# lawfuyang/HobbyRenderer

Hardware: AMD Instinct MI355X
Metric: Mrays/s at 1920×1080, 8 spp, 4 bounces; 1/2/4/8 GPU scaling (higher is better)
Workload: dtype f32; 1 GPU; config 2: Cornell-box-class procedural scene (38 triangles, 9 instances, closed room, emissive quad + default sun), 1920x1080, 8 spp (accumulation indices 0..7), 4 bounces; frames_in_flight=2, serial_kernels=False, mode=default

## Files before the change

hobbyrenderer_amd/csrc/pt_capi.cpp:

```cpp
#include <mutex>

#include "pt_capi_internal.h"

using namespace hrt;
using namespace hrt::capi;

static std::mutex g_errMutex;
static std::string g_createError;

int capi::fail(HrptContext* ctx, int code, const std::string& msg)
{
    if (ctx) ctx->err = msg;
    else { std::lock_guard<std::mutex> l(g_errMutex); g_createError = msg; }
    return code;
}

int capi::realloc_image(HrptContext* c, DeviceBuffer<float4>& image, size_t bytes)
{
    HIP_TRY(c, image.alloc(bytes));
    HIP_TRY(c, hipMemsetAsync(image, 0, bytes, c->stream));
    return HRPT_OK;
}

int hrpt_create(const HrptDeviceDesc* desc, HrptContext** out)
// ... 170 lines not shown
    c->accelStructure = structure;
    return HRPT_OK;
} catch (...) { return caught(c, "hrpt_set_acceleration_structure"); }

int hrpt_set_bvh_builder(HrptContext* c, int builder)
try {
    if (!c) return HRPT_ERR_INVALID_ARGUMENT;
    if (builder != HRPT_BVH_BUILDER_HOST_SAH && builder != HRPT_BVH_BUILDER_GPU_LBVH && builder != HRPT_BVH_BUILDER_GPU_PLOC && builder != HRPT_BVH_BUILDER_AUTO) return fail(c, HRPT_ERR_INVALID_ARGUMENT, "hrpt_set_bvh_builder: unknown builder");
    c->bvhBuilder = builder;
    return HRPT_OK;
} catch (...) { return caught(c, "hrpt_set_bvh_builder"); }

int hrpt_get_build_info(HrptContext* c, HrptBuildInfo* out)
try {
    if (!c) return HRPT_ERR_INVALID_ARGUMENT;
    if (!out) return fail(c, HRPT_ERR_INVALID_ARGUMENT, "hrpt_get_build_info: null out");
    if (!c->haveScene) return fail(c, HRPT_ERR_INVALID_ARGUMENT, "hrpt_get_build_info: no scene uploaded");
    *out = c->buildInfo;
    return HRPT_OK;
} catch (...) { return caught(c, "hrpt_get_build_info"); }

int hrpt_get_stats(HrptContext* c, HrptStats* out)
try {
    if (!c) return HRPT_ERR_INVALID_ARGUMENT;
    if (!out) return fail(c, HRPT_ERR_INVALID_ARGUMENT, "hrpt_get_stats: null out");
    HIP_TRY(c, hipSetDevice(c->device));
    HIP_TRY(c, hipStreamSynchronize(c->stream));
    DeviceCounters h[kCounterShards];
    HIP_TRY(c, hipMemcpy(h, c->perContext.dCounters, sizeof h, hipMemcpyDeviceToHost));
    memset(out, 0, sizeof *out);
    DeviceCounters total{};
    for (int i = 0; i < kCounterShards; ++i) {
        total.closestRays += h[i].closestRays; total.shadowRays += h[i].shadowRays; total.paths += h[i].paths; total.neeEntries += h[i].neeEntries;
        total.neeSamples += h[i].neeSamples; total.radianceShade += h[i].radianceShade; total.radianceShadow += h[i].radianceShadow; total.skipped16 += h[i].skipped16;
        total.fusedPaths += h[i].fusedPaths; total.fusedEntries += h[i].fusedEntries;
    }
    out->closestRays = total.closestRays; out->shadowRays = total.shadowRays; out->paths = total.paths;
    out->neeEntries = total.neeEntries; out->neeSamples = total.neeSamples;
    out->megakernelFallbacks = c->megakernelFallbacks; out->queuePoolBytes = c->wf.poolBytes;
    if (total.neeEntries || c->wf.raygenBytes || c->wf.resolveBytes) {
        wavefront_queue_bytes(c->wf, total, out->traceQueueBytes, out->shadeQueueBytes, out->shadowQueueBytes);
        out->raygenQueueBytes = c->wf.raygenBytes; out->resolveQueueBytes = c->wf.resolveBytes;
    }
    if (c->timed) { float ms = 0.0f; if (hipEventElapsedTime(&ms, c->evStart, c->evStop) == hipSuccess) out->lastRenderMs = ms; }
    wavefront_collect_timing(c->wf);
    out->traceKernelMs = c->wf.kernelMs[kKernelExtend]; out->traceKernelLaunches = c->wf.kernelLaunches[kKernelExtend];
    out->shadeKernelMs = c->wf.kernelMs[kKernelShade]; out->shadeKernelLaunches = c->wf.kernelLaunches[kKernelShade];
    out->shadowKernelMs = c->wf.kernelMs[kKernelShadow]; out->shadowKernelLaunches = c->wf.kernelLaunches[kKernelShadow];
    out->raygenKernelMs = c->wf.kernelMs[kKernelRaygen]; out->raygenKernelLaunches = c->wf.kernelLaunches[kKernelRaygen];
    out->resolveKernelMs = c->wf.kernelMs[kKernelResolve]; out->resolveKernelLaunches = c->wf.kernelLaunches[kKernelResolve];
    out->bvhNodeCount = c->bvhNodes; out->bvhTriangleCount = c->bvhTris; out->bvhMaxDepth = c->traits.bvhMaxDepth;
    return HRPT_OK;
} catch (...) { return caught(c, "hrpt_get_stats"); }

int hrpt_reset_stats(HrptContext* c)
try {
    if (!c) return HRPT_ERR_INVALID_ARGUMENT;
    HIP_TRY(c, hipSetDevice(c->device));
    HIP_TRY(c, hipStreamSynchronize(c->stream));
    HIP_TRY(c, hipMemsetAsync(c->perContext.dCounters, 0, sizeof(DeviceCounters) * kCounterShards, c->stream));
    wavefront_reset_timing(c->wf);
    c->megakernelFallbacks = 0;
    return HRPT_OK;
} catch (...) { return caught(c, "hrpt_reset_stats"); }
```

hobbyrenderer_amd/csrc/pt_kernels.h:

```cpp
#pragma once

#include <hip/hip_runtime.h>
#include <stdint.h>

#include "../../include/hobbyrt_pt.h"

namespace hrt {

struct SceneView;
struct MotionArgs;
struct GpuNode4; struct GpuNodeQ;

constexpr int kCounterShards = 32;
struct DeviceCounters {
    unsigned long long closestRays;
    unsigned long long shadowRays;
    unsigned long long paths;
    unsigned long long neeEntries;
    unsigned long long neeSamples;
    unsigned long long radianceShade;
    unsigned long long radianceShadow;
    unsigned long long skipped16;
    unsigned long long fusedPaths;
    unsigned long long fusedEntries;
};

struct TileRect {
    uint32_t x0, y0, x1, y1;
    uint32_t stripeCount = 1, stripeIndex = 0;
    __host__ __device__ uint32_t columns() const { uint32_t all = (x1 - x0 + 7u) / 8u; return all > stripeIndex ? (all - stripeIndex + stripeCount - 1u) / stripeCount : 0u; }
    __host__ __device__ uint32_t column_x(uint32_t k) const { return x0 + (k * stripeCount + stripeIndex) * 8u; }
};

hipError_t launch_megakernel(const SceneView& scene, const HrptPathTracerConstants& constants, float4* accumulation,
                             float4* output, uint32_t imageWidth, TileRect rect, DeviceCounters* counters, hipStream_t stream);

hipError_t launch_gbuffer_megakernel(const SceneView& scene, const HrptPathTracerConstants& constants, float4* const* planes, uint32_t planeMask,
                                     uint32_t imageWidth, TileRect rect, hipStream_t stream);

hipError_t launch_motion_megakernel(const SceneView& scene, const HrptPathTracerConstants& constants, float4* const* planes, uint32_t planeMask,
                                    const MotionArgs& motion, uint32_t imageWidth, TileRect rect, hipStream_t stream);

hipError_t launch_post_chain(const float4* hdr, float4* display, uint32_t pixelCount, const HrptPostParams& params, uint32_t* histogram,
                             float* exposure, hipStream_t stream);

size_t bloom_pyramid_words(uint32_t width, uint32_t height);
bool bloom_params_valid(const HrptBloomParams& params);
hipError_t launch_bloom(float4* hdr, uint32_t width, uint32_t height, const HrptBloomParams& params, uint32_t* downPyramid, uint32_t* upPyramid,
                        uint32_t tailTexels, hipStream_t stream);
void bloom_pack_probe(const float* rgb, uint32_t count, uint32_t* packed, float* unpacked);
void bloom_host(const float* hdrIn, float* hdrOut, uint32_t width, uint32_t height, const HrptBloomParams& params, int nthreads);

bool temporal_params_valid(const HrptTemporalParams& params);
hipError_t launch_temporal(const HrptTemporalImages& images, uint32_t width, uint32_t height, const HrptPlanarViewConstants& view,
                           const HrptPlanarViewConstants& prevView, const HrptTemporalParams& params, hipStream_t stream);
// ... 44 lines not shown
```

hobbyrenderer_amd/csrc/pt_wavefront.hip:

```cpp
#define HRPT_PHASE_TU 1
#include "pt_wavefront.h"

#include <mutex>
#include <type_traits>
#include <unordered_map>
#include <vector>

#include "bvh_build.h"
#include "pt_gbuffer.h"
#include "pt_motion.h"
#include "pt_path.h"

#ifdef HRPT_PHASE_PROFILE
__device__ unsigned long long g_phaseCounters[128];
#endif
#ifdef HRPT_SKY_DEBUG
__device__ float g_skyDebug[2048 * 16];
#endif

namespace hrt {

namespace {

#include "pt_wf_common.h"
// ... 184 lines not shown
        float t = 0.0f;
        if (hipEventElapsedTime(&t, st.events[i], st.events[i + 1]) == hipSuccess) { st.kernelMs[st.kind[i / 2]] += t; st.kernelLaunches[st.kind[i / 2]]++; }
    }
    st.eventsUsed = 0;
}

#ifdef HRPT_SKY_DEBUG
extern "C" int hrpt_sky_debug_read(float* out) { return hipMemcpyFromSymbol(out, HIP_SYMBOL(g_skyDebug), sizeof(float) * 2048 * 16) == hipSuccess ? 0 : -3; }
#endif
#ifdef HRPT_PHASE_PROFILE
extern "C" int hrpt_phase_profile_read(unsigned long long* out128)
{
    if (hipMemcpyFromSymbol(out128, HIP_SYMBOL(g_phaseCounters), 128 * sizeof(unsigned long long)) != hipSuccess) return -3;
    static const unsigned long long zero[128] = { 0 };
    if (hipMemcpyToSymbol(HIP_SYMBOL(g_phaseCounters), zero, sizeof zero) != hipSuccess) return -3;
    return 0;
}
#endif

void wavefront_reset_timing(WavefrontState& st)
{
    st.eventsUsed = 0;
    for (int k = 0; k < kKernelClasses; ++k) { st.kernelMs[k] = 0.0f; st.kernelLaunches[k] = 0; }
    st.raygenBytes = 0; st.resolveBytes = 0;
}

void wavefront_queue_bytes(const WavefrontState& st, const DeviceCounters& c, uint64_t& trace, uint64_t& shade, uint64_t& shadow)
{
    const uint64_t path = st.plan.pathRecordBytes, survivors = c.closestRays > c.paths ? c.closestRays - c.paths : 0;
    trace = c.closestRays * (32 + 16);
    shade = c.closestRays * (path + 16) + survivors * path + c.neeEntries * 80 + c.neeSamples * 16 + c.radianceShade * 32;
    shadow = c.neeEntries * 48 + c.neeSamples * 16 + c.radianceShadow * (32 + 32);
    if (st.plan.shadowMode == kShadowSlim) {
        shade = c.closestRays * (path + 16) + survivors * path + c.neeEntries * 32 + c.radianceShade * 32;
        shadow = c.neeEntries * (32 + 16) + c.radianceShadow * (16 + 32);
    }
    if (st.plan.shadowMode == kShadowResolve) shadow += c.neeEntries * 32 + c.neeSamples * 16 + c.shadowRays * 72 + c.neeEntries * st.plan.maxLights * 8;
    if (st.plan.fusedPrimary) {
        trace -= c.paths * 16;
        shade = shade - c.paths * (path - 16) + c.paths * 16;
        shadow -= c.skipped16 * 16;
        trace -= c.fusedPaths * 32;
        shade = shade - c.fusedPaths * 32 + c.fusedEntries * 16;
    }
}

namespace {
bool timing_mark(WavefrontState& st, hipStream_t stream, KernelClass kind, bool begin)
{
    if (st.eventsUsed >= 4096) return true;
    if (st.eventsUsed + 1 > st.events.size()) {
        hipEvent_t e;
        if (hipEventCreate(&e) != hipSuccess) return false;
        st.events.push_back(e);
    }
    if (begin) { if (st.kind.size() < st.eventsUsed / 2 + 1) st.kind.resize(st.eventsUsed / 2 + 1); st.kind[st.eventsUsed / 2] = (uint8_t)kind; }
    (void)hipEventRecord(st.events[st.eventsUsed], stream);
    st.eventsUsed++;
    return true;
}
struct PoolCarver {
    char* base; size_t off = 0;
    template <class T> void operator()(T*& stream, size_t bytes, bool present = true)
    {
        stream = reinterpret_cast<T*>(reinterpret_cast<uintptr_t>(base) + (present ? off : 0));
        if (present) off += (bytes + 255) & ~(size_t)255;
    }
};
size_t counter_bytes(uint64_t capacity) { return (size_t)(capacity / 64) * 4; }
void carve_paths_and_hits(PoolCarver& carve, WfBuffers& b, int queues, uint64_t capacity, bool hasMedium, bool hasInstances)
{
    for (int p = 0; p < queues; ++p) {
        carve(b.rayO[p], capacity * 16); carve(b.rayD[p], capacity * 16); carve(b.thr[p], capacity * 16);
        carve(b.med0[p], capacity * 16, hasMedium); carve(b.med1[p], capacity * 16, hasMedium);
        carve(b.pathCnt[p], counter_bytes(capacity));
    }
    carve(b.hit, capacity * 16);
    carve(b.hitInst, capacity * 4, hasInstances); if (!hasInstances) b.hitInst = nullptr;
}
size_t carve_pool(char* base, WfArgs& a, uint64_t capacity, uint32_t maxLights, const SceneTraits& traits, bool hasInstances)
{
    const bool hasShadowRayQueue = traits.hasNonOpaque || maxLights > 1;
    PoolCarver carve{ base };
    WfBuffers& b = a.b;
    carve_paths_and_hits(carve, b, 2, capacity, traits.hasMedium, hasInstances);
    carve(a.primaryArgs, sizeof(PrimaryArgs));
    carve(b.sh0, capacity * 16); carve(b.sh1, capacity * 16); carve(b.sh2, capacity * 16); carve(b.sh3, capacity * 16); carve(b.sh4, capacity * 16);
    carve(b.shL, capacity * 16 * maxLights);
    carve(b.shadowCnt, counter_bytes(capacity)); carve(b.radiance, capacity * 16);
    carve(b.sqO, capacity * 16 * maxLights, hasShadowRayQueue); carve(b.sqD, capacity * 16 * maxLights, hasShadowRayQueue); carve(b.sqId, capacity * 4 * maxLights, hasShadowRayQueue);
    carve(b.sqCnt, counter_bytes(capacity), hasShadowRayQueue); carve(b.shVis, capacity * 4 * maxLights, hasShadowRayQueue); carve(b.sqCand, capacity * 8 * kShadowCandidates * maxLights, hasShadowRayQueue);
    return carve.off;
}
size_t carve_gbuffer_pool(char* base, WfArgs& a, uint64_t capacity, bool hasMedium, bool hasInstances)
{
    PoolCarver carve{ base };
    carve_paths_and_hits(carve, a.b, 1, capacity, hasMedium, hasInstances);
    carve(a.b.radiance, capacity * 16);
    carve(a.counters, sizeof(DeviceCounters) * kCounterShards);
    return carve.off;
}
void fill_scene_args(WfArgs& a, const WavefrontState& st, const SceneView& scene, const SceneTraits& traits, TileRect rect, uint32_t width)
{
    a.scene = scene;
    a.tilesX = rect.columns(); a.tilesY = (rect.y1 - rect.y0 + 7) / 8; a.rect = rect; a.imageWidth = width; a.pixelsPadded = a.tilesX * a.tilesY * 64;
    a.hasMedium = traits.hasMedium ? 1u : 0u; a.hasStochasticAlpha = traits.hasStochasticAlpha ? 1u : 0u; a.allOpaque = traits.hasNonOpaque ? 0u : 1u;
    a.refillMin = st.knobs.refillMin ? st.knobs.refillMin : kRefillMinDefault; a.streamSegments = st.knobs.drainSegments ? 0u : 1u;
}
hipError_t size_batch_and_pool(WavefrontState& st, const RenderPlan& plan, const SceneTraits& traits, bool hasInstances, uint64_t pixelsPadded, uint32_t accumCount,
                               hipStream_t stream, WfArgs& a, uint32_t& sppPerBatch, std::string& error)
{
    sppPerBatch = accumCount < kMaxSppPerBatch ? accumCount : kMaxSppPerBatch;
    uint64_t maxSamples = 64ull << 20;
    if (pixelsPadded * sppPerBatch * plan.bytesPerSample > st.poolBytes) {
        size_t freeB = 0, totalB = 0;
        if (hipMemGetInfo(&freeB, &totalB) == hipSuccess) {
            const uint64_t budget = (uint64_t)(freeB + st.poolBytes) / 2;
            if (budget / plan.bytesPerSample < maxSamples) maxSamples = budget / plan.bytesPerSample;
        }
    }
// ... 153 lines not shown
```

hobbyrenderer_amd/csrc/pt_wf_common.h:

```cpp

constexpr uint32_t kMaxSppPerBatch = 64;

struct WfBuffers {
    float4 *rayO[2], *rayD[2], *thr[2], *med0[2], *med1[2];
    uint32_t* pathCnt[2];
    float4* hit;
    uint32_t* hitInst;
    float4 *sh0, *sh1, *sh2, *sh3, *sh4, *shL;
    uint32_t* shadowCnt;
    float4 *sqO, *sqD; uint32_t* sqId; uint32_t* sqCnt; uint32_t* shVis;
    uint2* sqCand;
    float4* radiance;
};

struct WfArgs {
    SceneView scene;
    WfBuffers b;
    uint32_t segSize;
    uint32_t numSegments;
    uint32_t numSamples;
    uint32_t pixelsPadded;
    uint32_t tilesX, tilesY;
    TileRect rect;
    uint32_t imageWidth;
    uint32_t spp;
    uint32_t maxLights;
    uint32_t hasMedium;
    uint32_t hasStochasticAlpha;
    uint32_t allOpaque;
    uint32_t refillMin;
    uint32_t streamSegments;
    uint32_t slimShadow;
    uint32_t shadowParity;
    uint32_t nodeLoopMin;
    uint32_t sortShade;
    uint32_t shadeInstances, shadeMaterials;
    const struct PrimaryArgs* primaryArgs;
    uint32_t primary;
    int32_t* spill[2];
    DeviceCounters* counters;
};
// ... 146 lines not shown
```

hobbyrenderer_amd/csrc/pt_wf_shade.h:

```cpp
template <int MAXL>
struct NeeBuf { float ux[MAXL], uy[MAXL]; uint32_t light[MAXL]; };

static_assert(sizeof(GpuTriAttr) == kTriAttrBytes && sizeof(GpuInstShade) == kInstShadeBytes && sizeof(HrptMaterialConstants) == kMaterialBytes, "pt_wavefront_plan.h shade_table_bytes");
HRT_DEV LdsShadeTables copy_shade_tables(char* dst, const WfArgs& a)
{
    const SceneView& s = a.scene;
    const uint32_t nA = s.triCount * (uint32_t)(sizeof(GpuTriAttr) / 16), nI = a.shadeInstances * (uint32_t)(sizeof(GpuInstShade) / 16);
    const uint32_t nM = a.shadeMaterials * (uint32_t)(sizeof(HrptMaterialConstants) / 4);
    float4* const dA = reinterpret_cast<float4*>(dst); float4* const dI = dA + nA; uint32_t* const dM = reinterpret_cast<uint32_t*>(dI + nI);
    const float4* const sA = reinterpret_cast<const float4*>(s.attrs); const float4* const sI = reinterpret_cast<const float4*>(s.instShade);
    const uint32_t* const sM = reinterpret_cast<const uint32_t*>(s.materials);
    for (uint32_t i = threadIdx.x; i < nA; i += kBlock) dA[i] = sA[i];
    for (uint32_t i = threadIdx.x; i < nI; i += kBlock) dI[i] = sI[i];
    for (uint32_t i = threadIdx.x; i < nM; i += kBlock) dM[i] = sM[i];
    LdsShadeTables t;
    t.attrs = (uint32_t)(uintptr_t)(LdsShadeTables::LdsPtr)dst; t.instShade = t.attrs + nA * 16u; t.materials = t.instShade + nI * 16u;
    return t;
}


struct ShadeLane { bool valid, inA; uint32_t slot; float4 o, d, t, ha; };
struct ShadeWave { uint32_t outCount = 0, shCount = 0, ringHead = 0, pending = 0; unsigned int nEntriesOut = 0, nRadiance = 0; };
template <int MAXL, bool SIMPLE, bool PRIMARY, uint32_t RING, bool FUSED, class TABLES>
HRT_DEV void shade_iteration(const WfArgs& a, const HrptPathTracerConstants& cb, const TABLES& tables, float* const ring, uint32_t in, uint32_t out, int bounce, int lastBounce,
                             const ShadeLane& L, uint32_t baseA, uint32_t baseB, bool endsA, ShadeWave& w, uint32_t& outCountB, uint32_t& shCountB)
{
    static_assert(!FUSED || (PRIMARY && SIMPLE && MAXL == 1), "wf_bounce0: the bounce-0 SIMPLE single-light body");
    static_assert((RING & (RING - 1u)) == 0u && RING >= 1u && RING <= 64u, "ring positions are masked; one flush takes at most 64 entries");
    constexpr uint32_t kRing = RING;
    const SceneView& s = a.scene;
    const uint32_t lane = lane_id();
    const bool inA = L.inA;
    uint32_t& outCount = w.outCount; uint32_t& shCount = w.shCount;
    outCountB = 0; shCountB = 0;
            bool valid = L.valid, alive = false, wantDefer = false, wantRadiance = false;
            LobeDraw ld; ld.spec = false; ld.specProb = 0.0f; ld.root = 0.0f; ld.sp = 0.0f; ld.cp = 0.0f;
            uint32_t nNee = 0, smp = 0, slotIn = 0;
            PathState ps; f3 neeT = mk3(0.0f, 0.0f, 0.0f);
            constexpr bool STREAMED = MAXL == 0;
            NeeBuf<(STREAMED ? 1 : MAXL)> nee; SurfaceCarry carry;
            if (valid) {
                HRT_PHASE(PH_SHADE_ITER);
                const uint32_t slot = L.slot;
                slotIn = slot;
                const float4 o = L.o, d = L.d, t = L.t, ha = L.ha;
                uint32_t tri = __float_as_uint(ha.w);
                const bool noPath = PRIMARY && tri == kNoPathRecord;
                if (tri < kNoPathRecord) tri &= 0x1FFFFFFFu;
                ps.ray.o = mk3(o.x, o.y, o.z); ps.ray.d = mk3(d.x, d.y, d.z); ps.ray.tmin = o.w; ps.ray.tmax = 1e10f;
                ps.rng = __float_as_uint(d.w);
                ps.throughput = mk3(t.x, t.y, t.z); smp = __float_as_uint(t.w);
                ps.radiance = mk3(0.0f, 0.0f, 0.0f);
                if (!SIMPLE && a.hasMedium) {
                    float4 m0 = a.b.med0[in][slot], m1 = a.b.med1[in][slot];
                    ps.sigmaA = mk3(m0.x, m0.y, m0.z); ps.interiorIOR = m0.w; ps.sigmaS = mk3(m1.x, m1.y, m1.z); ps.inVolume = m1.w != 0.0f;
                } else { ps.sigmaA = mk3(0.0f, 0.0f, 0.0f); ps.sigmaS = mk3(0.0f, 0.0f, 0.0f); ps.interiorIOR = 1.0f; ps.inVolume = false; }
                bool addRadiance = false; f3 add = mk3(0.0f, 0.0f, 0.0f);
                if (noPath) {
                } else if (tri != 0xFFFFFFFFu) {
                    HRT_PHASE(PH_SHADE_HIT);
// ... 27 lines not shown
                        g[6] = cb.m_SunDirection[0]; g[7] = cb.m_SunDirection[1]; g[8] = cb.m_SunDirection[2]; g[9] = s.lights[0].m_Intensity;
                        g[10] = ps.radiance.x; g[11] = ps.radiance.y; g[12] = ps.radiance.z; g[13] = ps.throughput.x; g[14] = ps.throughput.y; g[15] = ps.throughput.z;
                    }
#endif
                }
                if constexpr (PRIMARY) {
                    a.b.radiance[smp] = addRadiance ? make_float4(0.0f + add.x, 0.0f + add.y, 0.0f + add.z, 0.0f) : make_float4(0.0f, 0.0f, 0.0f, 0.0f);
                } else if (addRadiance) {
                    float4 r = a.b.radiance[smp];
                    r.x = r.x + add.x; r.y = r.y + add.y; r.z = r.z + add.z;
                    a.b.radiance[smp] = r;
                }
                if (lastBounce) alive = false;
                wantRadiance = addRadiance && !PRIMARY;
            }
            w.nRadiance += (unsigned int)__popcll(__ballot(wantRadiance));
            const unsigned long long mA = __ballot(alive && inA), mB = __ballot(alive && !inA);
            if (alive) {
                HRT_PHASE(PH_SHADE_WRITE);
                uint32_t o = inA ? baseA + outCount + prefix_rank(mA) : baseB + prefix_rank(mB);
                a.b.rayO[out][o] = make_float4(ps.ray.o.x, ps.ray.o.y, ps.ray.o.z, ps.ray.tmin);
                a.b.rayD[out][o] = make_float4(ps.ray.d.x, ps.ray.d.y, ps.ray.d.z, __uint_as_float(ps.rng));
                a.b.thr[out][o] = make_float4(ps.throughput.x, ps.throughput.y, ps.throughput.z, __uint_as_float(smp));
                if (!SIMPLE && a.hasMedium) {
                    a.b.med0[out][o] = make_float4(ps.sigmaA.x, ps.sigmaA.y, ps.sigmaA.z, ps.interiorIOR);
                    a.b.med1[out][o] = make_float4(ps.sigmaS.x, ps.sigmaS.y, ps.sigmaS.z, ps.inVolume ? 1.0f : 0.0f);
                }
            }
            const unsigned long long msA = __ballot(nNee > 0 && inA), msB = __ballot(nNee > 0 && !inA);
            if (SIMPLE && MAXL == 1 && a.slimShadow && nNee > 0) {
                uint32_t e = inA ? baseA + shCount + prefix_rank(msA) : baseB + prefix_rank(msB);
                a.b.sh0[e] = make_float4(carry.worldPos.x, carry.worldPos.y, carry.worldPos.z, __uint_as_float(slotIn));
                a.b.sh1[e] = make_float4(carry.N.x, carry.N.y, carry.N.z, __uint_as_float(carry.material));
                if constexpr (FUSED) a.b.rayD[in][slotIn] = L.d;
            } else if (nNee > 0) {
                uint32_t e = inA ? baseA + shCount + prefix_rank(msA) : baseB + prefix_rank(msB);
                a.b.sh0[e] = make_float4(carry.worldPos.x, carry.worldPos.y, carry.worldPos.z, __uint_as_float(smp));
                a.b.sh1[e] = make_float4(carry.N.x, carry.N.y, carry.N.z, carry.roughness);
                a.b.sh2[e] = make_float4(carry.V.x, carry.V.y, carry.V.z, carry.metallic);
                a.b.sh3[e] = make_float4(carry.baseColor.x, carry.baseColor.y, carry.baseColor.z, carry.ior);
                a.b.sh4[e] = make_float4(neeT.x, neeT.y, neeT.z, __uint_as_float(nNee));
                if (STREAMED) {
                    const f3 sunDir = mk3(cb.m_SunDirection[0], cb.m_SunDirection[1], cb.m_SunDirection[2]);
                    uint32_t rng = carry.rngBeforeLights, j = 0;
                    for (uint32_t i = 0; i < cb.m_LightCount; ++i) {
                        HrptGPULight l = load_light(s, i);
                        float ux, uy;
                        if (nee_draw<false>(l, carry.N, carry.worldPos, sunDir, rng, ux, uy)) a.b.shL[(size_t)e * a.maxLights + j++] = make_float4(ux, uy, __uint_as_float(i), 0.0f);
                    }
                } else {
#pragma unroll
                    for (int j = 0; j < (STREAMED ? 1 : MAXL); ++j)
                        if ((uint32_t)j < nNee) a.b.shL[(size_t)e * a.maxLights + j] = make_float4(nee.ux[j], nee.uy[j], __uint_as_float(nee.light[j]), 0.0f);
                }
            }
            outCount += (uint32_t)__popcll(mA); shCount += (uint32_t)__popcll(msA);
            outCountB = (uint32_t)__popcll(mB); shCountB = (uint32_t)__popcll(msB);
            w.nEntriesOut += (unsigned int)(__popcll(msA) + __popcll(msB));
            if (SIMPLE) {
                const unsigned long long md = __ballot(wantDefer);
                const uint32_t nNew = (uint32_t)__popcll(md);
                uint32_t first = 0;
                bool parked = false;
                for (int round = 0; round < (kRing < 64u ? 3 : 2) && !parked; ++round) {
                uint32_t nPark = nNew - first;
                if (w.pending + nPark <= kRing) parked = true;
                else nPark = (kRing < 64u && w.pending == 0u) ? kRing : 0u;
// ... 97 lines not shown
            if (SORT && a.sortShade && haveSeg) permuted = sort_segment(segBase, cnt, permBase + permSel * segSize);
        };
        open_segment();
        while (haveSeg) {
            const uint32_t takeA = cnt - next < 64u ? cnt - next : 64u;
            const uint32_t segA = seg, baseA = segBase, nextA = next;
            const bool endsA = nextA + takeA >= cnt;
            uint32_t takeB = 0, segB = 0, baseB = 0, cntB = 0;
            if (endsA && takeA < 64u) {
                uint32_t probe = seg + totalWaves;
                for (; probe < a.numSegments; probe += totalWaves) {
                    cntB = uniform(PRIMARY ? path_count(a, in, probe) : a.b.pathCnt[in][probe]);
                    if (cntB) break;
                    if (lane == 0) { a.b.pathCnt[out][probe] = 0; a.b.shadowCnt[probe] = 0; }
                }
                if (probe < a.numSegments) {
                    segB = probe; baseB = probe * a.segSize; takeB = cntB < 64u - takeA ? cntB : 64u - takeA;
                    if (SORT && a.sortShade) permutedB = sort_segment(baseB, cntB, permBase + (permSel ^ 1u) * segSize);
                } else segB = probe;
            }
            ShadeLane L; L.valid = lane < takeA + takeB; L.inA = lane < takeA; L.slot = 0;
            if (L.valid) {
                const uint32_t slot = L.inA ? baseA + ((SORT && permuted) ? (uint32_t)permBase[permSel * segSize + nextA + lane] : nextA + lane)
                                          : baseB + ((SORT && permutedB) ? (uint32_t)permBase[(permSel ^ 1u) * segSize + (lane - takeA)] : lane - takeA);
                L.slot = slot;
                if constexpr (PRIMARY) {
                    const PrimaryArgs& pr = *a.primaryArgs;
                    L.o = make_float4(pr.cam[0], pr.cam[1], pr.cam[2], 0.0f); L.d = a.b.rayD[in][slot];
                    L.t = make_float4(1.0f, 1.0f, 1.0f, __uint_as_float(slot));
                } else { L.o = a.b.rayO[in][slot]; L.d = a.b.rayD[in][slot]; L.t = a.b.thr[in][slot]; }
                L.ha = a.b.hit[slot];
            }
            uint32_t outCountB = 0, shCountB = 0;
            if constexpr (LDS_TABLES) shade_iteration<MAXL, SIMPLE, PRIMARY, kShadeRing, false>(a, cb, ldsTables, ring, in, out, bounce, lastBounce, L, baseA, baseB, endsA, w, outCountB, shCountB);
            else shade_iteration<MAXL, SIMPLE, PRIMARY, kShadeRing, false>(a, cb, globalTables, ring, in, out, bounce, lastBounce, L, baseA, baseB, endsA, w, outCountB, shCountB);
            if (!endsA) next = nextA + takeA;
            else {
                if (lane == 0) { a.b.pathCnt[out][segA] = outCount; a.b.shadowCnt[segA] = shCount; }
                if (takeB) {
                    seg = segB; segBase = baseB; cnt = cntB; next = takeB;
                    outCount = outCountB; shCount = shCountB;
                    haveSeg = true;
                    if (SORT) { permSel ^= 1u; permuted = permutedB; permutedB = false; }
                    if (next >= cnt) {
                        if (lane == 0) { a.b.pathCnt[out][seg] = outCount; a.b.shadowCnt[seg] = shCount; }
                        seg += totalWaves; open_segment();
                    }
                } else if (takeA < 64u) { seg = segB; haveSeg = false; }
                else { seg += totalWaves; open_segment(); }
            }
        }
    }
    block_count_add_uniform<2>(a.counters, { 3, 5 }, { w.nEntriesOut, w.nRadiance });
}
template <int MAXL, bool SIMPLE, bool PRIMARY = false>
__global__ __launch_bounds__(kBlock) __attribute__((amdgpu_waves_per_eu(kWavesShade, kWavesShade))) void wf_shade(WfArgs a, HrptPathTracerConstants cb, uint32_t parity, int bounce, int lastBounce)
{
    shade_paths<MAXL, SIMPLE, PRIMARY, false>(a, cb, parity, bounce, lastBounce);
}
template <int MAXL, bool SIMPLE, bool PRIMARY = false>
__global__ __launch_bounds__(kBlock) __attribute__((amdgpu_waves_per_eu(kWavesShade, kWavesShade))) void wf_shade_lt(WfArgs a, HrptPathTracerConstants cb, uint32_t parity, int bounce, int lastBounce)
{
    shade_paths<MAXL, SIMPLE, PRIMARY, true>(a, cb, parity, bounce, lastBounce);
}

template <int DEPTH>
__global__ __launch_bounds__(kBlock) __attribute__((amdgpu_waves_per_eu(kWavesShade, kWavesShade))) void wf_bounce0(WfArgs a, HrptPathTracerConstants cb, int lastBounce)
{
// ... 32 lines not shown
            int32_t cur = (!active || emptyScene || !finite) ? kTraversalDone : (s.nodeCount == 0 ? s.rootLeaf : 0);
            active = cur != kTraversalDone;
            while (__ballot(active) != 0ull) {
                if (active) {
                    while (cur >= 0) {
                        cur = inner_step(lbvh, cur, noi, inv, r.tmin, tlim, stack, sp);
                        if ((uint32_t)__popcll(__ballot(cur >= 0)) < a.nodeLoopMin) break;
                    }
                    if (cur < 0 && cur != kTraversalDone) {
                        const uint32_t enc = (uint32_t)(~cur), first = enc >> 2, count = (enc & 3u) + 1u;
                        for (uint32_t i = 0; i < count; ++i) {
                            float4 ta, tb, tc; lbvh.tri(first + i, ta, tb, tc);
                            float t, u, v;
                            if (tri_test(mk3(ta.x, ta.y, ta.z), mk3(tb.x, tb.y, tb.z), mk3(tc.x, tc.y, tc.z), r, sh, t, u, v)) {
                                const uint32_t inst = __float_as_uint(ta.w), prim = __float_as_uint(tb.w);
                                const bool takeHit = !best.valid || key_less(t, inst, prim, best.t, best.inst, best.prim);
                                best.t = takeHit ? t : best.t; best.u = takeHit ? u : best.u; best.v = takeHit ? v : best.v;
                                best.inst = takeHit ? inst : best.inst; best.prim = takeHit ? prim : best.prim; best.tri = takeHit ? first + i : best.tri;
                                best.opaque = takeHit ? (__float_as_uint(tc.w) & 7u) : best.opaque;
                                best.valid = best.valid || takeHit;
                                tlim = takeHit ? t : tlim;
                            }
                        }
                        cur = sp == 0 ? kTraversalDone : stack.pop(--sp);
                    }
                    active = cur != kTraversalDone;
                }
            }
            L.o = make_float4(pr.cam[0], pr.cam[1], pr.cam[2], 0.0f);
            L.d = make_float4(r.d.x, r.d.y, r.d.z, __uint_as_float(rng));
            L.t = make_float4(1.0f, 1.0f, 1.0f, __uint_as_float(L.slot));
            L.ha = make_float4(best.t, best.u, best.v, __uint_as_float(!havePath ? kNoPathRecord : (best.valid ? (best.tri | ((best.opaque >> 1) << 29)) : 0xFFFFFFFFu)));
            uint32_t outCountB, shCountB;
            shade_iteration<1, true, true, kBounce0Ring, true>(a, cb, ldsTables, ring, 0u, 1u, 0, lastBounce, L, segBase, segBase, next + take >= cnt, w, outCountB, shCountB);
        }
        if (lane == 0) { a.b.pathCnt[1][seg] = w.outCount; a.b.shadowCnt[seg] = w.shCount; }
    }
    block_count_add(&a.counters->closestRays, 0, nRays);
    __syncthreads();
    block_count_add(&a.counters->closestRays, 2, nRays);
    __syncthreads();
    block_count_add(&a.counters->closestRays, 8, nRays);
    block_count_add_uniform<3>(a.counters, { 3, 5, 9 }, { w.nEntriesOut, w.nRadiance, w.nEntriesOut });
}
```

hobbyrenderer_amd/csrc/pt_wf_shadow.h:

```cpp
template <bool DIRONLY>
__global__ __launch_bounds__(kBlock) void wf_shadow_rays(WfArgs a, HrptPathTracerConstants cb)
{
    const SceneView& s = a.scene;
    const f3 sunDir = mk3(cb.m_SunDirection[0], cb.m_SunDirection[1], cb.m_SunDirection[2]);
    const uint32_t wavesPerBlock = kBlock / 64, lane = lane_id();
    const uint32_t gw = uniform(blockIdx.x * wavesPerBlock + (threadIdx.x >> 6)), totalWaves = gridDim.x * wavesPerBlock;
    for (uint32_t seg = gw; seg < a.numSegments; seg += totalWaves) {
        const uint32_t cnt = uniform(a.b.shadowCnt[seg]), segBase = seg * a.segSize, items = cnt * a.maxLights;
        uint32_t outCount = 0;
        for (uint32_t i0 = 0; i0 < items; i0 += 64) {
            const uint32_t i = i0 + lane;
            bool valid = false; Ray ray; uint32_t id = 0;
            if (i < items) {
                HRT_PHASE(PH_SHADOW_RAYS_ITEM);
                const uint32_t el = i / a.maxLights, j = i - el * a.maxLights, e = segBase + el;
                id = e * a.maxLights + j;
                float4 h4 = a.b.sh4[e];
                if (j < __float_as_uint(h4.w)) {
                    float4 h0 = a.b.sh0[e], h1 = a.b.sh1[e], ls = a.b.shL[(size_t)e * a.maxLights + j];
                    HrptGPULight l = load_light(s, __float_as_uint(ls.z));
                    f3 L; float maxDist;
                    if (nee_direction<DIRONLY>(l, mk3(h1.x, h1.y, h1.z), mk3(h0.x, h0.y, h0.z), sunDir, cb.m_CosSunAngularRadius, ls.x, ls.y, L, maxDist)) {
                        ray = shadow_ray(mk3(h0.x, h0.y, h0.z), L, maxDist);
                        valid = true;
// ... 6 lines not shown
                const uint32_t o = segBase * a.maxLights + outCount + prefix_rank(m);
                a.b.sqO[o] = make_float4(ray.o.x, ray.o.y, ray.o.z, ray.tmin);
                a.b.sqD[o] = make_float4(ray.d.x, ray.d.y, ray.d.z, ray.tmax);
                a.b.sqId[o] = id;
            }
            outCount += (uint32_t)__popcll(m);
        }
        if (lane == 0) a.b.sqCnt[seg] = outCount;
    }
}

template <bool LDS_BVH, int DEPTH, int W, bool DIRONLY, int MODE, int TL = 0>
__global__ __launch_bounds__(kBlock) __attribute__((amdgpu_waves_per_eu(MODE == 2 && TL == 0 ? 4 : ((MODE == 1 || TL != 0) ? 3 : 1)))) void wf_shadow(WfArgs a, HrptPathTracerConstants cb, int bounce)
{
    static_assert(!TL || (!LDS_BVH && W == 4 && (MODE == kShadowOpaque || MODE == kShadowSlim)), "two-level structure: opaque any-hit query over the global tree");
    static_assert(W != kQuantisedTree || (!LDS_BVH && !TL), "quantised nodes: flat tree in global memory");
    constexpr bool NONOPAQUE = MODE == kShadowBuffered || MODE == kShadowResolve;
    constexpr bool SLIM = MODE == kShadowSlim;
    constexpr int kLdsMax = MODE == kShadowResolve ? kExtendLdsStack : kShadowLdsStack;
    extern __shared__ __attribute__((aligned(128))) char smem[];
    LdsStack<DEPTH, kLdsMax> stack; LdsBvh<W> lbvh;
    constexpr size_t candBytes = MODE == kShadowBuffered ? (size_t)kShadowCandidates * 2 * kBlock * 4 : 0;
    setup_lds<LDS_BVH, DEPTH, W>(smem, a.scene, stack, lbvh, candBytes);
    if (DEPTH > kLdsMax) { stack.spill = a.spill[1] + blockIdx.x * kBlock + threadIdx.x; stack.spillStride = gridDim.x * kBlock; }
    LdsCandidates cand; cand.base = reinterpret_cast<int32_t*>(smem + (size_t)LdsStack<DEPTH, kLdsMax>::kRows * kBlock * 4) + threadIdx.x;
    LdsCandidates3 cand3; cand3.base = cand.base;
    typename GlobalBvhOf<(TL ? kTwoLevelTree : W)>::type gbvh = GlobalBvhOf<(TL ? kTwoLevelTree : W)>::make(a.scene);
    const SceneView& s = a.scene;
    const f3 sunDir = mk3(cb.m_SunDirection[0], cb.m_SunDirection[1], cb.m_SunDirection[2]);
    const float sunIntensity = s.lights[0].m_Intensity;

    const uint32_t wavesPerBlock = kBlock / 64, lane = lane_id();
    const uint32_t gw = uniform(blockIdx.x * wavesPerBlock + (threadIdx.x >> 6)), totalWaves = gridDim.x * wavesPerBlock;
    unsigned int nRays = 0, nSamples = 0, nRadiance = 0, nSkipped16 = 0;
    auto process = [&](uint32_t e) {
                HRT_PHASE(PH_SHADOW_ENTRY);
                if (SLIM) {
                    const float4 h0 = a.b.sh0[e], h1 = a.b.sh1[e];
                    const uint32_t slot = __float_as_uint(h0.w);
                    const float4 rd = a.b.rayD[a.shadowParity][slot];
                    const f3 origin = mk3(h0.x, h0.y, h0.z), N = mk3(h1.x, h1.y, h1.z);
                    uint32_t rng = __float_as_uint(rd.w);
                    const float ux = hrt_rng_next(&rng), uy = hrt_rng_next(&rng);
                    ++nSamples;
                    HrptGPULight l = load_light(s, 0u);
                    f3 L; float maxDist;
                    if (!nee_direction<true>(l, N, origin, sunDir, cb.m_CosSunAngularRadius, ux, uy, L, maxDist)) return;
                    float shadow;
                    if (LDS_BVH) shadow = shadow_query<true>(s, lbvh, origin, L, maxDist, stack);
                    else if constexpr (TL == 2) shadow = shadow_query_two_level_buffered<kTwoLevelCandidates>(s, gbvh, shadow_ray(origin, L, maxDist), stack, cand3);
                    else shadow = shadow_query<true>(s, gbvh, origin, L, maxDist, stack);
                    ++nRays;
                    if (shadow != 0.0f) {
                        const float4 th = a.primary ? make_float4(1.0f, 1.0f, 1.0f, __uint_as_float(slot)) : a.b.thr[a.shadowParity][slot];
                        if (a.primary) ++nSkipped16;
                        const HrptMaterialConstants& mat = s.materials[__float_as_uint(h1.w)];
                        f3 dif, spec;
                        nee_contribution<true>(s, l, nee_lighting(N, mk3(-rd.x, -rd.y, -rd.z), mk3(mat.m_BaseColor), hrt_max(mat.m_RoughnessMetallic[0], 0.04f),
                                                                  mat.m_RoughnessMetallic[1], mat.m_IOR), origin, sunDir, sunIntensity, L, dif, spec);
                        f3 totalDiffuse = mk3(0.0f, 0.0f, 0.0f) + dif * shadow, totalSpecular = mk3(0.0f, 0.0f, 0.0f);
                        if (bounce == 0) totalSpecular = totalSpecular + spec * shadow;
                        const f3 dsum = totalDiffuse + (bounce == 0 ? totalSpecular : mk3(0.0f, 0.0f, 0.0f));
                        if (dsum.x != 0.0f || dsum.y != 0.0f || dsum.z != 0.0f) {
                            const f3 term = mk3(th.x, th.y, th.z) * dsum;
                            const uint32_t smp = __float_as_uint(th.w);
                            float4 r = a.b.radiance[smp];
                            r.x = r.x + term.x; r.y = r.y + term.y; r.z = r.z + term.z;
                            a.b.radiance[smp] = r;
                            ++nRadiance;
                        }
                    }
                    return;
                }
                float4 h0 = a.b.sh0[e], h1 = a.b.sh1[e], h4 = a.b.sh4[e];
                f3 origin = mk3(h0.x, h0.y, h0.z), N = mk3(h1.x, h1.y, h1.z), T = mk3(h4.x, h4.y, h4.z);
                uint32_t smp = __float_as_uint(h0.w), n = __float_as_uint(h4.w);
                nSamples += n;
                f3 totalDiffuse = mk3(0.0f, 0.0f, 0.0f), totalSpecular = mk3(0.0f, 0.0f, 0.0f);
                float4 ls0 = make_float4(0.0f, 0.0f, 0.0f, 0.0f);
                if (MODE != kShadowResolve && n) ls0 = a.b.shL[(size_t)e * a.maxLights];
                for (uint32_t j = 0; j < n; ++j) {
                    HRT_PHASE(PH_SHADOW_SAMPLE);
                    uint32_t vis = kVisCandidates;
                    if (MODE == kShadowResolve) {
                        vis = a.b.shVis[e * a.maxLights + j];
                        if (vis == kVisNoRay) continue;
                        if (vis == kVisBlocked) { ++nRays; continue; }
                    }
                    float4 ls = ls0;
                    if (MODE == kShadowResolve || j) ls = a.b.shL[(size_t)e * a.maxLights + j];
                    HrptGPULight l = load_light(s, __float_as_uint(ls.z));
// ... 29 lines not shown
                        if (bounce == 0) totalSpecular = totalSpecular + spec * shadow;
                    }
                }
                f3 dsum = totalDiffuse + (bounce == 0 ? totalSpecular : mk3(0.0f, 0.0f, 0.0f));
                if (dsum.x != 0.0f || dsum.y != 0.0f || dsum.z != 0.0f) {
                    f3 term = T * dsum;
                    float4 r = a.b.radiance[smp];
                    r.x = r.x + term.x; r.y = r.y + term.y; r.z = r.z + term.z;
                    a.b.radiance[smp] = r;
                    ++nRadiance;
                }
    };
    if (NONOPAQUE) {
        uint32_t seg = gw, cnt = 0, segBase = 0, next = 0; bool haveSeg = false;
        auto open_segment = [&]() {
            haveSeg = false; cnt = 0; next = 0;
            for (; seg < a.numSegments; seg += totalWaves) {
                cnt = uniform(a.b.shadowCnt[seg]);
                if (cnt) { segBase = seg * a.segSize; haveSeg = true; break; }
            }
        };
        open_segment();
        while (haveSeg) {
            uint32_t e = 0xFFFFFFFFu, filled = 0;
            while (filled < 64u && haveSeg) {
                uint32_t take = cnt - next < 64u - filled ? cnt - next : 64u - filled;
                if (lane >= filled && lane < filled + take) e = segBase + next + (lane - filled);
                next += take; filled += take;
                if (next >= cnt) { seg += totalWaves; open_segment(); }
            }
            if (e != 0xFFFFFFFFu) process(e);
        }
    } else {
        for (uint32_t seg = gw; seg < a.numSegments; seg += totalWaves) {
            const uint32_t cnt = uniform(a.b.shadowCnt[seg]), segBase = seg * a.segSize;
            for (uint32_t base = 0; base < cnt; base += 64) {
                uint32_t i = base + lane;
                if (i < cnt) process(segBase + i);
            }
        }
    }
    block_count_add(&a.counters->closestRays, 1, nRays);
    __syncthreads();
    block_count_add(&a.counters->closestRays, 4, nSamples);
    __syncthreads();
    block_count_add(&a.counters->closestRays, 6, nRadiance);
    if (SLIM && a.primary) { __syncthreads(); block_count_add(&a.counters->closestRays, 7, nSkipped16); }
}
```

Before: 27300 Mrays/s.

## Store shadow RNG per entry and recompute primary view dir in slim shadow pass

The slim shadow path now stores the RNG seed per shadow entry in a dedicated array (aliased onto sh2) instead of gathering the full rayD float4 by slot. For primary bounces it recomputes the view direction with primary_ray only for lit samples, and it gathers rayD/throughput only on the non-primary lit path. The shade kernel no longer writes rayD in the fused bounce-0 variant. The non-compact shadow loop now preloads segment counts across 64 lanes and skips empty segments with a ballot. These changes trade scattered 16-byte gathers for a 4-byte coalesced read plus some ALU, and the byte-accounting counters are updated to match.

Result: no change. 27540 Mrays/s, median of 6 (+0.9%).

```diff
diff --git a/hobbyrenderer_amd/csrc/pt_capi.cpp b/hobbyrenderer_amd/csrc/pt_capi.cpp
--- a/hobbyrenderer_amd/csrc/pt_capi.cpp
+++ b/hobbyrenderer_amd/csrc/pt_capi.cpp
@@ -226,7 +226,7 @@
     DeviceCounters total{};
     for (int i = 0; i < kCounterShards; ++i) {
         total.closestRays += h[i].closestRays; total.shadowRays += h[i].shadowRays; total.paths += h[i].paths; total.neeEntries += h[i].neeEntries;
-        total.neeSamples += h[i].neeSamples; total.radianceShade += h[i].radianceShade; total.radianceShadow += h[i].radianceShadow; total.skipped16 += h[i].skipped16;
+        total.neeSamples += h[i].neeSamples; total.radianceShade += h[i].radianceShade; total.radianceShadow += h[i].radianceShadow; total.slimGathers += h[i].slimGathers;
         total.fusedPaths += h[i].fusedPaths; total.fusedEntries += h[i].fusedEntries;
     }
     out->closestRays = total.closestRays; out->shadowRays = total.shadowRays; out->paths = total.paths;
diff --git a/hobbyrenderer_amd/csrc/pt_kernels.h b/hobbyrenderer_amd/csrc/pt_kernels.h
--- a/hobbyrenderer_amd/csrc/pt_kernels.h
+++ b/hobbyrenderer_amd/csrc/pt_kernels.h
@@ -20,7 +20,7 @@
     unsigned long long neeSamples;
     unsigned long long radianceShade;
     unsigned long long radianceShadow;
-    unsigned long long skipped16;
+    unsigned long long slimGathers;
     unsigned long long fusedPaths;
     unsigned long long fusedEntries;
 };
diff --git a/hobbyrenderer_amd/csrc/pt_wavefront.hip b/hobbyrenderer_amd/csrc/pt_wavefront.hip
--- a/hobbyrenderer_amd/csrc/pt_wavefront.hip
+++ b/hobbyrenderer_amd/csrc/pt_wavefront.hip
@@ -240,16 +240,15 @@
     shade = c.closestRays * (path + 16) + survivors * path + c.neeEntries * 80 + c.neeSamples * 16 + c.radianceShade * 32;
     shadow = c.neeEntries * 48 + c.neeSamples * 16 + c.radianceShadow * (32 + 32);
     if (st.plan.shadowMode == kShadowSlim) {
-        shade = c.closestRays * (path + 16) + survivors * path + c.neeEntries * 32 + c.radianceShade * 32;
-        shadow = c.neeEntries * (32 + 16) + c.radianceShadow * (16 + 32);
+        shade = c.closestRays * (path + 16) + survivors * path + c.neeEntries * 36 + c.radianceShade * 32;
+        shadow = c.neeEntries * 36 + c.slimGathers * 32 + c.radianceShadow * 32;
     }
     if (st.plan.shadowMode == kShadowResolve) shadow += c.neeEntries * 32 + c.neeSamples * 16 + c.shadowRays * 72 + c.neeEntries * st.plan.maxLights * 8;
     if (st.plan.fusedPrimary) {
         trace -= c.paths * 16;
         shade = shade - c.paths * (path - 16) + c.paths * 16;
-        shadow -= c.skipped16 * 16;
         trace -= c.fusedPaths * 32;
-        shade = shade - c.fusedPaths * 32 + c.fusedEntries * 16;
+        shade -= c.fusedPaths * 32;
     }
 }
 
@@ -294,6 +293,7 @@
     carve_paths_and_hits(carve, b, 2, capacity, traits.hasMedium, hasInstances);
     carve(a.primaryArgs, sizeof(PrimaryArgs));
     carve(b.sh0, capacity * 16); carve(b.sh1, capacity * 16); carve(b.sh2, capacity * 16); carve(b.sh3, capacity * 16); carve(b.sh4, capacity * 16);
+    b.shRng = reinterpret_cast<uint32_t*>(b.sh2);
     carve(b.shL, capacity * 16 * maxLights);
     carve(b.shadowCnt, counter_bytes(capacity)); carve(b.radiance, capacity * 16);
     carve(b.sqO, capacity * 16 * maxLights, hasShadowRayQueue); carve(b.sqD, capacity * 16 * maxLights, hasShadowRayQueue); carve(b.sqId, capacity * 4 * maxLights, hasShadowRayQueue);
diff --git a/hobbyrenderer_amd/csrc/pt_wf_common.h b/hobbyrenderer_amd/csrc/pt_wf_common.h
--- a/hobbyrenderer_amd/csrc/pt_wf_common.h
+++ b/hobbyrenderer_amd/csrc/pt_wf_common.h
@@ -7,6 +7,7 @@
     float4* hit;
     uint32_t* hitInst;
     float4 *sh0, *sh1, *sh2, *sh3, *sh4, *shL;
+    uint32_t* shRng;
     uint32_t* shadowCnt;
     float4 *sqO, *sqD; uint32_t* sqId; uint32_t* sqCnt; uint32_t* shVis;
     uint2* sqCand;
diff --git a/hobbyrenderer_amd/csrc/pt_wf_shade.h b/hobbyrenderer_amd/csrc/pt_wf_shade.h
--- a/hobbyrenderer_amd/csrc/pt_wf_shade.h
+++ b/hobbyrenderer_amd/csrc/pt_wf_shade.h
@@ -21,11 +21,10 @@
 
 struct ShadeLane { bool valid, inA; uint32_t slot; float4 o, d, t, ha; };
 struct ShadeWave { uint32_t outCount = 0, shCount = 0, ringHead = 0, pending = 0; unsigned int nEntriesOut = 0, nRadiance = 0; };
-template <int MAXL, bool SIMPLE, bool PRIMARY, uint32_t RING, bool FUSED, class TABLES>
+template <int MAXL, bool SIMPLE, bool PRIMARY, uint32_t RING, class TABLES>
 HRT_DEV void shade_iteration(const WfArgs& a, const HrptPathTracerConstants& cb, const TABLES& tables, float* const ring, uint32_t in, uint32_t out, int bounce, int lastBounce,
                              const ShadeLane& L, uint32_t baseA, uint32_t baseB, bool endsA, ShadeWave& w, uint32_t& outCountB, uint32_t& shCountB)
 {
-    static_assert(!FUSED || (PRIMARY && SIMPLE && MAXL == 1), "wf_bounce0: the bounce-0 SIMPLE single-light body");
     static_assert((RING & (RING - 1u)) == 0u && RING >= 1u && RING <= 64u, "ring positions are masked; one flush takes at most 64 entries");
     constexpr uint32_t kRing = RING;
     const SceneView& s = a.scene;
@@ -119,7 +118,7 @@
                 uint32_t e = inA ? baseA + shCount + prefix_rank(msA) : baseB + prefix_rank(msB);
                 a.b.sh0[e] = make_float4(carry.worldPos.x, carry.worldPos.y, carry.worldPos.z, __uint_as_float(slotIn));
                 a.b.sh1[e] = make_float4(carry.N.x, carry.N.y, carry.N.z, __uint_as_float(carry.material));
-                if constexpr (FUSED) a.b.rayD[in][slotIn] = L.d;
+                a.b.shRng[e] = __float_as_uint(L.d.w);
             } else if (nNee > 0) {
                 uint32_t e = inA ? baseA + shCount + prefix_rank(msA) : baseB + prefix_rank(msB);
                 a.b.sh0[e] = make_float4(carry.worldPos.x, carry.worldPos.y, carry.worldPos.z, __uint_as_float(smp));
@@ -283,8 +282,8 @@
                 L.ha = a.b.hit[slot];
             }
             uint32_t outCountB = 0, shCountB = 0;
-            if constexpr (LDS_TABLES) shade_iteration<MAXL, SIMPLE, PRIMARY, kShadeRing, false>(a, cb, ldsTables, ring, in, out, bounce, lastBounce, L, baseA, baseB, endsA, w, outCountB, shCountB);
-            else shade_iteration<MAXL, SIMPLE, PRIMARY, kShadeRing, false>(a, cb, globalTables, ring, in, out, bounce, lastBounce, L, baseA, baseB, endsA, w, outCountB, shCountB);
+            if constexpr (LDS_TABLES) shade_iteration<MAXL, SIMPLE, PRIMARY, kShadeRing>(a, cb, ldsTables, ring, in, out, bounce, lastBounce, L, baseA, baseB, endsA, w, outCountB, shCountB);
+            else shade_iteration<MAXL, SIMPLE, PRIMARY, kShadeRing>(a, cb, globalTables, ring, in, out, bounce, lastBounce, L, baseA, baseB, endsA, w, outCountB, shCountB);
             if (!endsA) next = nextA + takeA;
             else {
                 if (lane == 0) { a.b.pathCnt[out][segA] = outCount; a.b.shadowCnt[segA] = shCount; }
@@ -383,7 +382,7 @@
             L.t = make_float4(1.0f, 1.0f, 1.0f, __uint_as_float(L.slot));
             L.ha = make_float4(best.t, best.u, best.v, __uint_as_float(!havePath ? kNoPathRecord : (best.valid ? (best.tri | ((best.opaque >> 1) << 29)) : 0xFFFFFFFFu)));
             uint32_t outCountB, shCountB;
-            shade_iteration<1, true, true, kBounce0Ring, true>(a, cb, ldsTables, ring, 0u, 1u, 0, lastBounce, L, segBase, segBase, next + take >= cnt, w, outCountB, shCountB);
+            shade_iteration<1, true, true, kBounce0Ring>(a, cb, ldsTables, ring, 0u, 1u, 0, lastBounce, L, segBase, segBase, next + take >= cnt, w, outCountB, shCountB);
         }
         if (lane == 0) { a.b.pathCnt[1][seg] = w.outCount; a.b.shadowCnt[seg] = w.shCount; }
     }
diff --git a/hobbyrenderer_amd/csrc/pt_wf_shadow.h b/hobbyrenderer_amd/csrc/pt_wf_shadow.h
--- a/hobbyrenderer_amd/csrc/pt_wf_shadow.h
+++ b/hobbyrenderer_amd/csrc/pt_wf_shadow.h
@@ -62,15 +62,14 @@
 
     const uint32_t wavesPerBlock = kBlock / 64, lane = lane_id();
     const uint32_t gw = uniform(blockIdx.x * wavesPerBlock + (threadIdx.x >> 6)), totalWaves = gridDim.x * wavesPerBlock;
-    unsigned int nRays = 0, nSamples = 0, nRadiance = 0, nSkipped16 = 0;
+    unsigned int nRays = 0, nSamples = 0, nRadiance = 0, nGathered = 0;
     auto process = [&](uint32_t e) {
                 HRT_PHASE(PH_SHADOW_ENTRY);
                 if (SLIM) {
                     const float4 h0 = a.b.sh0[e], h1 = a.b.sh1[e];
+                    uint32_t rng = a.b.shRng[e];
                     const uint32_t slot = __float_as_uint(h0.w);
-                    const float4 rd = a.b.rayD[a.shadowParity][slot];
                     const f3 origin = mk3(h0.x, h0.y, h0.z), N = mk3(h1.x, h1.y, h1.z);
-                    uint32_t rng = __float_as_uint(rd.w);
                     const float ux = hrt_rng_next(&rng), uy = hrt_rng_next(&rng);
                     ++nSamples;
                     HrptGPULight l = load_light(s, 0u);
@@ -82,11 +81,19 @@
                     else shadow = shadow_query<true>(s, gbvh, origin, L, maxDist, stack);
                     ++nRays;
                     if (shadow != 0.0f) {
-                        const float4 th = a.primary ? make_float4(1.0f, 1.0f, 1.0f, __uint_as_float(slot)) : a.b.thr[a.shadowParity][slot];
-                        if (a.primary) ++nSkipped16;
+                        f3 V; float4 th;
+                        if (a.primary) {
+                            f3 po, pd; uint32_t seed;
+                            (void)primary_ray(a, *a.primaryArgs, slot, po, pd, seed);
+                            V = mk3(-pd.x, -pd.y, -pd.z); th = make_float4(1.0f, 1.0f, 1.0f, __uint_as_float(slot));
+                        } else {
+                            const float4 rd = a.b.rayD[a.shadowParity][slot];
+                            V = mk3(-rd.x, -rd.y, -rd.z); th = a.b.thr[a.shadowParity][slot];
+                            ++nGathered;
+                        }
                         const HrptMaterialConstants& mat = s.materials[__float_as_uint(h1.w)];
                         f3 dif, spec;
-                        nee_contribution<true>(s, l, nee_lighting(N, mk3(-rd.x, -rd.y, -rd.z), mk3(mat.m_BaseColor), hrt_max(mat.m_RoughnessMetallic[0], 0.04f),
+                        nee_contribution<true>(s, l, nee_lighting(N, V, mk3(mat.m_BaseColor), hrt_max(mat.m_RoughnessMetallic[0], 0.04f),
                                                                   mat.m_RoughnessMetallic[1], mat.m_IOR), origin, sunDir, sunIntensity, L, dif, spec);
                         f3 totalDiffuse = mk3(0.0f, 0.0f, 0.0f) + dif * shadow, totalSpecular = mk3(0.0f, 0.0f, 0.0f);
                         if (bounce == 0) totalSpecular = totalSpecular + spec * shadow;
@@ -182,11 +189,16 @@
             if (e != 0xFFFFFFFFu) process(e);
         }
     } else {
-        for (uint32_t seg = gw; seg < a.numSegments; seg += totalWaves) {
-            const uint32_t cnt = uniform(a.b.shadowCnt[seg]), segBase = seg * a.segSize;
-            for (uint32_t base = 0; base < cnt; base += 64) {
-                uint32_t i = base + lane;
-                if (i < cnt) process(segBase + i);
+        for (uint32_t seg0 = gw; seg0 < a.numSegments; seg0 += 64u * totalWaves) {
+            const uint32_t mine = seg0 + lane * totalWaves;
+            const uint32_t myCnt = mine < a.numSegments ? a.b.shadowCnt[mine] : 0u;
+            for (unsigned long long left = __ballot(myCnt != 0u); left != 0ull; left &= left - 1ull) {
+                const uint32_t k = (uint32_t)__builtin_ctzll(left);
+                const uint32_t cnt = (uint32_t)__builtin_amdgcn_readlane((int)myCnt, (int)k), segBase = (seg0 + k * totalWaves) * a.segSize;
+                for (uint32_t base = 0; base < cnt; base += 64) {
+                    uint32_t i = base + lane;
+                    if (i < cnt) process(segBase + i);
+                }
             }
         }
     }
@@ -195,5 +207,5 @@
     block_count_add(&a.counters->closestRays, 4, nSamples);
     __syncthreads();
     block_count_add(&a.counters->closestRays, 6, nRadiance);
-    if (SLIM && a.primary) { __syncthreads(); block_count_add(&a.counters->closestRays, 7, nSkipped16); }
+    if (SLIM) { __syncthreads(); block_count_add(&a.counters->closestRays, 7, nGathered); }
 }
```
